# pyannote/pyannote-video

Hardware: AMD Instinct MI355X
Metric: frames/sec end-to-end detect->embed->cluster, 1080p@25fps (higher is better)
Workload: dtype f32 (detector scores, embedder) / f64 (tracker, clustering) / u8 frames; an f16 screening pass with a proven error bound decides which windows the detector's exact f32 chain is evaluated for -- results identical to dense f32 scoring (`dense_scoring`)

## Files before the change

pyannote-video_amd/csrc/ctx.hip:

```cpp
#include "pvf_internal.h"
#include "detect_ml.h"
#include <cmath>
#include <fstream>
#include <mutex>
#include <dlfcn.h>

static thread_local std::string g_err;
void pvf_set_error(const char* msg) { g_err = msg ? msg : ""; }
extern "C" const char* pvf_last_error(void) { return g_err.c_str(); }

static std::mutex g_ctx_mu;
static std::unordered_map<uint64_t, std::unique_ptr<Ctx>> g_ctxs;
static uint64_t g_next_ctx = 0x1000;

Ctx* pvf_ctx(pvf_handle h)
{
    std::lock_guard<std::mutex> lk(g_ctx_mu);
    auto it = g_ctxs.find(h);
    if (it == g_ctxs.end()) throw PvfError("unknown context handle");
    return it->second.get();
}

std::map<std::string, Tensor> pvf_read_container(const char* path)
{
// ... 216 lines not shown
        for (auto& pr : kv.second.pending) {
            float ms = 0;
            if (hipEventElapsedTime(&ms, pr.first, pr.second) == hipSuccess) kv.second.total_ms += ms;
            c->event_pool.push_back(pr.first);
            c->event_pool.push_back(pr.second);
        }
        kv.second.pending.clear();
    }
}

#define API_BEGIN try {
#define API_END                                                        \
    return 0;                                                          \
    }                                                                  \
    catch (const std::exception& e) { pvf_set_error(e.what()); return -1; } \
    catch (...) { pvf_set_error("unknown error"); return -2; }

extern "C" int32_t pvf_version(void) { return 500; }

extern "C" int32_t pvf_device_count(int32_t* n)
{
    API_BEGIN
    int k = 0;
    hipError_t e = hipGetDeviceCount(&k);
    if (e != hipSuccess) k = 0;
    *n = k;
    API_END
}

extern "C" int32_t pvf_ctx_create_prio(int32_t device, int32_t priority_class, pvf_handle* out)
{
    API_BEGIN
    int k = 0;
    if (hipGetDeviceCount(&k) != hipSuccess || k <= 0) throw PvfError("no HIP device visible: libpvface has no CPU fallback");
    PVF_REQUIRE(device >= 0 && device < k, "device index out of range");
    HIP_CHECK(hipSetDevice(device));
    hipDeviceProp_t prop;
    HIP_CHECK(hipGetDeviceProperties(&prop, device));
    if (strncmp(prop.gcnArchName, "gfx950", 6) != 0)
        throw PvfError(std::string("libpvface is built for gfx950 (MI355X) only; device is ") + prop.gcnArchName);
    std::unique_ptr<Ctx> c(new Ctx());
    c->device = device;
    c->n_cu = prop.multiProcessorCount;
    {
        int lo = 0, hi = 0;
        HIP_CHECK(hipDeviceGetStreamPriorityRange(&lo, &hi));
        int prio = priority_class < 0 ? lo : hi;
        if (const char* e = getenv("PVF_MAIN_STREAM_PRIO")) prio = (strcmp(e, "low") == 0) ? lo : hi;
        HIP_CHECK(hipStreamCreateWithPriority(&c->stream, hipStreamNonBlocking, priority_class == 2 ? lo : prio));
        HIP_CHECK(hipStreamCreateWithPriority(&c->det_stream, hipStreamNonBlocking, priority_class == 2 ? hi : lo));
    }
    if (const char* e = getenv("PVF_DETECTOR_SCREENING")) c->det_screen = atoi(e) != 0;
    if (const char* e = getenv("PVF_EMBEDDER_SPLIT")) c->emb_split = atoi(e) != 0;
    std::lock_guard<std::mutex> lk(g_ctx_mu);
    uint64_t id = g_next_ctx++;
    g_ctxs[id] = std::move(c);
    *out = id;
    API_END
}

extern "C" int32_t pvf_ctx_create(int32_t device, pvf_handle* out) { return pvf_ctx_create_prio(device, 0, out); }

extern "C" int32_t pvf_ctx_destroy(pvf_handle h)
{
    API_BEGIN
    Ctx* c = pvf_ctx(h);
    HIP_CHECK(hipSetDevice(c->device));
    (void)hipStreamSynchronize(c->stream);
    (void)hipStreamSynchronize(c->det_stream);
    for (auto& kv : c->frames) if (kv.second.owned) (void)hipFree((void*)kv.second.d);
    for (auto& kv : c->trackers) {
        Tracker& t = *kv.second;
        if (t.share) { if (--*t.share > 0) continue; delete t.share; t.share = nullptr; }
        if (t.d_state) (void)hipFree(t.d_state);
    }
    for (auto p : c->tracker_pool) (void)hipFree(p);
    for (int k = 0; k < 2; ++k) if (c->det_ev[k]) (void)hipEventDestroy(c->det_ev[k]);
    ml_plans_free(c);
    ingest_free_all(c);
    render_free_all(c);
    for (auto& kv : c->frame_pool) for (auto q : kv.second) {
        if (q.free_after) (void)hipEventDestroy(q.free_after);
        if (q.free_after_det) (void)hipEventDestroy(q.free_after_det);
        (void)hipFree(q.p);
    }
    if (c->d_orient_lut) (void)hipFree(c->d_orient_lut);
    if (c->d_wrap_lut) (void)hipFree(c->d_wrap_lut);
    (void)hipStreamDestroy(c->stream);
    (void)hipStreamDestroy(c->det_stream);
    std::lock_guard<std::mutex> lk(g_ctx_mu);
    g_ctxs.erase(h);
    API_END
}

extern "C" int32_t pvf_sync(pvf_handle h)
{
    API_BEGIN
    Ctx* c = pvf_ctx(h);
    std::lock_guard<std::recursive_mutex> det_lock(c->det_mu);
    std::lock_guard<std::recursive_mutex> api_lock(c->api_mu);
    HIP_CHECK(hipStreamSynchronize(c->det_stream));
    HIP_CHECK(hipStreamSynchronize(c->stream));
    API_END
}

extern "C" int32_t pvf_load_detector(pvf_handle h, const char* path)
// ... 219 lines not shown
```

pyannote-video_amd/csrc/pvf_internal.h:

```cpp
#pragma once
#include <hip/hip_runtime.h>
#include <cstdint>
#include <cstdio>
#include <cstring>
#include <deque>
#include <map>
#include <atomic>
#include <memory>
#include <mutex>
#include <stdexcept>
#include <string>
#include <unordered_map>
#include <vector>
#include "../../include/pvface.h"

#define PVF_FHOG_STRIDE 32

struct PvfError : std::runtime_error { using std::runtime_error::runtime_error; };
struct CandOverflow : PvfError { int needed; explicit CandOverflow(int n) : PvfError("detector: candidate buffer overflow"), needed(n) {} };
struct ScreenRetry : PvfError { ScreenRetry() : PvfError("detector: screening pass gave up") {} };

#define HIP_CHECK(expr)                                                                              \
    do {                                                                                             \
        hipError_t _e = (expr);                                                                      \
// ... 160 lines not shown
constexpr size_t TRK_B = TRK_A + (size_t)32 * 64 * 64 * 2;
constexpr size_t TRK_AS = TRK_B + (size_t)64 * 64;
constexpr size_t TRK_BS = TRK_AS + (size_t)512 * 32 * 2;
constexpr size_t TRK_POS = TRK_BS + 32;
constexpr size_t TRK_DOUBLES = TRK_POS + 4;
constexpr size_t TRKF_PLANE = (size_t)64 * 64;
constexpr size_t TRKF_A = 5 * TRKF_PLANE * sizeof(float);
constexpr size_t TRKF_BYTES = TRKF_A + TRKF_PLANE;
#define TRKF_SLOT(q) ((((q) & 511) << 3) | ((q) >> 9))

struct ChipJob {
    const uint8_t* img; int h, w;
    int bx0, by0, sw, sh, levels;
    double m[4], b[2];
    int rows, cols;
    bool empty;
};
struct ChipDetails { double l, t, r, b, cs, sn; int rows, cols; };

struct Ctx {
    int device = 0;
    hipStream_t stream = nullptr;
    hipStream_t det_stream = nullptr;
    DetectorModel det;
    ShapeModel shape;
    EmbedModel emb;
    TrackerTables ttab;
    std::unordered_map<uint64_t, Frame> frames;
    std::unordered_map<uint64_t, std::unique_ptr<Tracker>> trackers;
    std::vector<double*> tracker_pool;
    std::atomic<uint64_t> next_id{1};
    std::recursive_mutex api_mu;
    std::recursive_mutex det_mu;
    std::mutex frames_mu;
    std::mutex prof_mu;
    bool prof_on = false;
    std::map<std::string, ProfFamily> prof;
    std::vector<hipEvent_t> event_pool;
    DevBuf s_grad, s_pyr, s_hist, s_norm, s_feat, s_cand, s_misc, s_chip, s_chip_pyr, s_act0, s_act1, s_act2, s_trk0, s_trk1, s_trk2, s_trkfeat, s_clu0, s_clu1;
    HostBuf h_cand, h_misc;
    StageRing stage;
    DevBuf s_cand2[2], s_fptr[2];
    HostBuf h_cand2[2], h_fptr[2];
    hipEvent_t det_ev[2] = {nullptr, nullptr};
    int det_slot = 0;
    int det_cand_cap = 8192;
    bool det_screen = true, det_screen_suspended = false, screen_attr_set = false;
    int screen_list_cap = 1 << 20;
    DevBuf s_screen;
    int64_t screen_batches = 0, screen_listed = 0, screen_retries = 0;
    double screen_pipe_err = -1;
    bool screen_pipe_flushes_subnormals = false;
    bool emb_split = true, emb_probe_done = false;
    DevBuf s_emb_flags, s_emb_redo;
    int64_t emb_split_faces = 0, emb_reruns = 0;
    double emb_pipe_err = -1;
    int n_cu = 256;
    struct PoolBuf { uint8_t* p; hipEvent_t free_after; hipEvent_t free_after_det; };
    std::map<size_t, std::deque<PoolBuf>> frame_pool;
    size_t frame_pool_bytes = 0;
    void* ingest_rings = nullptr;
    void* render_state = nullptr;
    struct MlPlanCache* ml_plans = nullptr;
    std::map<std::vector<int>, std::unique_ptr<DevBuf>> resize_tabs;
    const void* feat_ring_owner = nullptr;
    uint8_t* d_orient_lut = nullptr;
    uint8_t* d_wrap_lut = nullptr;
    DevBuf s_orb_set, s_orb_work;
    int orb_n = 0, orb_cap = 0;

    Frame frame(uint64_t id)
    {
        std::lock_guard<std::mutex> lk(frames_mu);
        auto it = frames.find(id);
        if (it == frames.end()) throw PvfError("unknown frame handle");
        Frame& f = it->second;
        if (f.ready) {
            HIP_CHECK(hipStreamWaitEvent(stream, f.ready, 0));
            HIP_CHECK(hipStreamWaitEvent(det_stream, f.ready, 0));
            (void)hipEventDestroy(f.ready);
            f.ready = nullptr;
        }
        return f;
    }
    uint8_t* take_frame_buffer(size_t bytes, hipStream_t writer)
    {
        PoolBuf b{nullptr, nullptr, nullptr};
        {
            std::lock_guard<std::mutex> lk(frames_mu);
            auto& v = frame_pool[bytes];
            if (!v.empty()) { b = v.front(); v.pop_front(); frame_pool_bytes -= bytes; }
        }
        if (!b.p) {
            HIP_CHECK(hipMalloc((void**)&b.p, bytes));
            return b.p;
        }
        for (hipEvent_t e : {b.free_after, b.free_after_det}) {
            if (!e) continue;
            if (writer) HIP_CHECK(hipStreamWaitEvent(writer, e, 0));
            else HIP_CHECK(hipEventSynchronize(e));
            (void)hipEventDestroy(e);
        }
        return b.p;
    }
    void pool_give(uint8_t* p, size_t bytes)
    {
        hipEvent_t e = nullptr, e2 = nullptr;
// ... 86 lines not shown
```

pyannote-video_amd/csrc/resnet.hip:

```cpp
#include "pvf_internal.h"
#include <cmath>
#include <cstdlib>
#include <cstring>
#include <vector>

typedef float f32x4 __attribute__((ext_vector_type(4)));
typedef uint32_t u32x4 __attribute__((ext_vector_type(4)));
typedef float f32x16 __attribute__((ext_vector_type(16)));
typedef _Float16 f16x8 __attribute__((ext_vector_type(8)));
typedef _Float16 f16x2 __attribute__((ext_vector_type(2)));
typedef uint32_t u32x2 __attribute__((ext_vector_type(2)));

void face_chip_details(const EmbedModel& m, const int32_t* pts, ChipDetails* out)
{
    const double size = m.chip_size, padding = m.chip_padding;
    double fx[51], fy[51], tx[51], ty[51];
    int n = 0;
    for (int i = 17; i < 68; ++i) {
        if ((55 <= i && i <= 59) || (65 <= i && i <= 67)) continue;
        if (17 <= i && i <= 26) continue;
        fx[n] = ((padding + (double)m.mean_shape[2 * (i - 17)]) / (2 * padding + 1)) * size;
        fy[n] = ((padding + (double)m.mean_shape[2 * (i - 17) + 1]) / (2 * padding + 1)) * size;
        tx[n] = pts[2 * i]; ty[n] = pts[2 * i + 1];
        ++n;
    }
    double mfx = 0, mfy = 0, mtx = 0, mty = 0;
    for (int i = 0; i < n; ++i) { mfx += fx[i]; mfy += fy[i]; mtx += tx[i]; mty += ty[i]; }
    mfx /= n; mfy /= n; mtx /= n; mty /= n;
    double a = 0, b = 0, s = 0;
    for (int i = 0; i < n; ++i) {
        const double ax = fx[i] - mfx, ay = fy[i] - mfy, bx = tx[i] - mtx, by = ty[i] - mty;
        a += ax * bx + ay * by;
        b += ax * by - ay * bx;
        s += ax * ax + ay * ay;
    }
    const double ca = a / s, cb = b / s;
    const double scale = std::sqrt(ca * ca + cb * cb);
    const double hx = size / 2.0, hy = size / 2.0;
    const double cx = (ca * (hx - mfx) - cb * (hy - mfy)) + mtx;
    const double cy = (cb * (hx - mfx) + ca * (hy - mfy)) + mty;
    const double wv = size * scale;
    out->l = cx - wv / 2; out->t = cy - wv / 2; out->r = cx + wv / 2; out->b = cy + wv / 2;
    out->cs = ca / scale; out->sn = cb / scale;
    out->rows = m.chip_size; out->cols = m.chip_size;
}

struct ConvArgs {
    const float* in; int B, H, W, Cin;
    const float* w; int K;
    const float* frag;
    const float* bias; const float* gamma; const float* beta;
    float* out; int OH, OW, Cout;
    int AH, AW;
    int ksz, stride, pad;
    int skip_mode;
    const float* skip; int XH, XW, XC, SH, SW;
    const uint32_t* wsplit; float out_scale; int* flags;
};


__device__ __forceinline__ int small_div(int x, int d, float rd)
{
    int q = (int)((float)x * rd);
    const int r = x - q * d;
    q += (r >= d) ? 1 : 0;
    q -= (r < 0) ? 1 : 0;
    return q;
}

template <int WM, int WN>
__device__ __forceinline__ void conv_epilogue(const ConvArgs& a, float* smem, const f32x16& acc0, const f32x16& acc1, long M, long m0, int n0,
                                              int rel0, int b_first, int hw, float r_hw, float r_ow, int wave, int lane)
{
    constexpr int PITCH = 36;
    const int wm = wave / WN, wn = wave % WN;
    const int li = lane & 31, kh = lane >> 5;
    const int col = n0 + wn * 32 + li;
    const float bias = a.bias[col], g = a.gamma[col], bt = a.beta[col];
    if (a.AH == a.OH && a.AW == a.OW && a.skip_mode != 2) {
        float* T = smem + wave * 64 * PITCH;
#pragma unroll
        for (int t = 0; t < 2; ++t)
#pragma unroll
            for (int reg = 0; reg < 16; ++reg)
                T[(t * 32 + (reg & 3) + 8 * (reg >> 2) + 4 * kh) * PITCH + li] = (t == 0 ? acc0[reg] : acc1[reg]);
        __builtin_amdgcn_wave_barrier();
        const int c4 = lane & 7, cb = n0 + wn * 32 + 4 * c4;
        const float4 bias4 = *reinterpret_cast<const float4*>(a.bias + cb), g4 = *reinterpret_cast<const float4*>(a.gamma + cb),
                     bt4 = *reinterpret_cast<const float4*>(a.beta + cb);
#pragma unroll
        for (int it = 0; it < 8; ++it) {
            const int row = it * 8 + (lane >> 3);
            const long m = m0 + wm * 64 + row;
            if (m >= M) continue;
            const float4 x = *reinterpret_cast<const float4*>(&T[row * PITCH + 4 * c4]);
            float4 v = make_float4((x.x + bias4.x) * g4.x + bt4.x, (x.y + bias4.y) * g4.y + bt4.y, (x.z + bias4.z) * g4.z + bt4.z,
                                   (x.w + bias4.w) * g4.w + bt4.w);
            if (a.skip_mode == 1) {
                const float4 sk = *reinterpret_cast<const float4*>(a.skip + (size_t)m * a.Cout + cb);
                v.x += sk.x; v.y += sk.y; v.z += sk.z; v.w += sk.w;
            }
            { v.x = v.x < 0.0f ? 0.0f : v.x; v.y = v.y < 0.0f ? 0.0f : v.y; v.z = v.z < 0.0f ? 0.0f : v.z; v.w = v.w < 0.0f ? 0.0f : v.w; }
            *reinterpret_cast<float4*>(a.out + (size_t)m * a.Cout + cb) = v;
        }
        return;
    }
#pragma unroll
    for (int t = 0; t < 2; ++t)
#pragma unroll
        for (int reg = 0; reg < 16; ++reg) {
            const int row = (reg & 3) + 8 * (reg >> 2) + 4 * kh;
            const long m = m0 + wm * 64 + t * 32 + row;
            if (m >= M) continue;
            const int rel = rel0 + wm * 64 + t * 32 + row;
            const int bb = small_div(rel, hw, r_hw);
            const int rem = rel - bb * hw;
            const int oy = small_div(rem, a.OW, r_ow);
            const int ox = rem - oy * a.OW;
            const int b = b_first + bb;
            float v = 0.0f;
            if (oy < a.AH && ox < a.AW) v = ((t == 0 ? acc0[reg] : acc1[reg]) + bias) * g + bt;
            if (a.skip_mode == 1) v += a.skip[(size_t)m * a.Cout + col];
            else if (a.skip_mode == 2) {
                if (col < a.XC && oy < a.SH && ox < a.SW) {
                    const float* q = a.skip + (((size_t)b * a.XH + 2 * oy) * a.XW + 2 * ox) * a.XC + col;
                    v += (((q[0] + q[a.XC]) + q[(size_t)a.XW * a.XC]) + q[(size_t)a.XW * a.XC + a.XC]) * 0.25f;
                }
            }
            if (v < 0.0f) v = 0.0f;
            a.out[(size_t)m * a.Cout + col] = v;
        }
}

template <int WM, int WN>
__global__ void __launch_bounds__(256) conv_mfma_k(ConvArgs a)
{
    constexpr int BM = 64 * WM, BN = 32 * WN, KC = 32, PITCH = 36;
    static_assert(WM * WN == 4, "four waves per block");
    constexpr int SM_ROWS = (BM + BN > 256) ? BM + BN : 256;
    __shared__ __attribute__((aligned(16))) float smem[SM_ROWS * PITCH];
    float* As = smem;
    float* Bs = smem + BM * PITCH;
    const int tid = threadIdx.x, lane = tid & 63, wave = tid >> 6;
    const int wm = wave / WN, wn = wave % WN;
    const long M = (long)a.B * a.OH * a.OW;
    const long m0 = (long)blockIdx.x * BM;
    const int n0 = blockIdx.y * BN;
    f32x16 acc0, acc1;
#pragma unroll
    for (int i = 0; i < 16; ++i) { acc0[i] = 0.0f; acc1[i] = 0.0f; }

    constexpr int A_F4 = BM * 8 / 256, B_F4 = BN * 8 / 256;
    constexpr int RSRC_FLAGS = 0x00020000;
    constexpr int OOB = (int)0x80000000;
    const int hw = a.OH * a.OW;
    const int b_first = (int)(m0 / hw);
    const int rel0 = (int)(m0 - (long)b_first * hw);
    const float r_hw = 1.0f / (float)hw, r_ow = 1.0f / (float)a.OW;
    const size_t face = (size_t)a.H * a.W * a.Cin;
    const size_t in_bytes = (size_t)(a.B - b_first) * face * sizeof(float);
    const __amdgpu_buffer_rsrc_t rs_in = __builtin_amdgcn_make_buffer_rsrc((void*)(a.in + (size_t)b_first * face), 0,
                                                                           in_bytes > 0x7ffffff0u ? 0x7ffffff0 : (int)in_bytes, RSRC_FLAGS);
    int pa_off[A_F4], pa_y[A_F4], pa_x[A_F4];
#pragma unroll
    for (int q = 0; q < A_F4; ++q) {
        const int i = (tid + q * 256) >> 3;
        const long m = m0 + i;
        pa_off[q] = 0; pa_y[q] = -(1 << 20); pa_x[q] = 0;
        if (m < M) {
            const int rel = rel0 + i;
            const int bb = small_div(rel, hw, r_hw);
            const int rem = rel - bb * hw;
            const int oy = small_div(rem, a.OW, r_ow);
            const int ox = rem - oy * a.OW;
            if (oy < a.AH && ox < a.AW) {
                pa_y[q] = oy * a.stride - a.pad; pa_x[q] = ox * a.stride - a.pad;
                pa_off[q] = ((bb * a.H + pa_y[q]) * a.W + pa_x[q]) * a.Cin;
            }
        }
    }
    const int Kpad = (a.K + KC - 1) / KC * KC;
    const int j4 = tid & 7;
    const float* wrow[B_F4];
// ... 18 lines not shown
        if (f_k + KC < Kpad) {
            f_k += KC;
            f_c += KC;
            if (f_c >= a.Cin) { f_c = 0; if (++f_s == a.ksz) { f_s = 0; ++f_r; } }
        }
    };
    auto issue = [&]() {
#pragma unroll
        for (int q = 0; q < A_F4; ++q) va[q] = __builtin_amdgcn_raw_buffer_load_b128(rs_in, voff[q], 0, 0);
#pragma unroll
        for (int q = 0; q < B_F4; ++q) vb[q] = *reinterpret_cast<const float4*>(wrow[q] + woff);
    };
    auto park = [&]() {
#pragma unroll
        for (int q = 0; q < A_F4; ++q) {
            uint32_t* row = reinterpret_cast<uint32_t*>(&As[((tid + q * 256) >> 3) * PITCH + 2 * j4]);
            *reinterpret_cast<uint2*>(row) = make_uint2(va[q].x, va[q].z);
            *reinterpret_cast<uint2*>(row + 16) = make_uint2(va[q].y, va[q].w);
        }
#pragma unroll
        for (int q = 0; q < B_F4; ++q) {
            float* row = &Bs[((tid + q * 256) >> 3) * PITCH + 2 * j4];
            *reinterpret_cast<float2*>(row) = make_float2(vb[q].x, vb[q].z);
            *reinterpret_cast<float2*>(row + 16) = make_float2(vb[q].y, vb[q].w);
        }
    };
    const int li = lane & 31, kh = lane >> 5;
    const float* pa0 = &As[(wm * 64 + li) * PITCH + 16 * kh];
    const float* pa1 = pa0 + 32 * PITCH;
    const float* pb = &Bs[(wn * 32 + li) * PITCH + 16 * kh];
    offsets();
    issue();
    offsets();
    for (int k0 = 0; k0 < Kpad; k0 += KC) {
        park();
        __syncthreads();
        issue();
        __builtin_amdgcn_sched_barrier(0);
        offsets();
        f32x4 fa0[4], fa1[4], fb[4];
#pragma unroll
        for (int q = 0; q < 4; ++q) {
            fa0[q] = *reinterpret_cast<const f32x4*>(pa0 + 4 * q);
            fa1[q] = *reinterpret_cast<const f32x4*>(pa1 + 4 * q);
            fb[q] = *reinterpret_cast<const f32x4*>(pb + 4 * q);
        }
#pragma unroll
        for (int s = 0; s < 16; ++s) {
            acc0 = __builtin_amdgcn_mfma_f32_32x32x2f32(fa0[s >> 2][s & 3], fb[s >> 2][s & 3], acc0, 0, 0, 0);
            acc1 = __builtin_amdgcn_mfma_f32_32x32x2f32(fa1[s >> 2][s & 3], fb[s >> 2][s & 3], acc1, 0, 0, 0);
        }
        __syncthreads();
    }
    conv_epilogue<WM, WN>(a, smem, acc0, acc1, M, m0, n0, rel0, b_first, hw, r_hw, r_ow, wave, lane);
}


#define EMB_A_SCALE_EXP 8
#define EMB_F16_LIMIT 65504.0f

__global__ void __launch_bounds__(256) conv_wsplit_k(const float* __restrict__ w, int total, int w_exp, _Float16* __restrict__ out)
{
    const int i = blockIdx.x * 256 + threadIdx.x;
    if (i >= total) return;
    const float v = ldexpf(w[i], w_exp);
    const _Float16 hi = (_Float16)v;
    const _Float16 lo = (_Float16)(v - (float)hi);
    const int row32 = i >> 5, kk = i & 31;
    out[(size_t)row32 * 64 + kk] = hi;
    out[(size_t)row32 * 64 + 32 + kk] = lo;
}

template <int WM, int WN>
__global__ void __launch_bounds__(256) conv_split_k(ConvArgs a)
{
    constexpr int BM = 64 * WM, BN = 32 * WN, KC = 32, PITCH = 36;
    static_assert(WM * WN == 4, "four waves per block");
    constexpr int SM_ROWS = (BM + BN > 256) ? BM + BN : 256;
    __shared__ __attribute__((aligned(16))) float smem[SM_ROWS * PITCH];
    uint32_t* As = reinterpret_cast<uint32_t*>(smem);
    uint32_t* Bs = As + BM * PITCH;
    const int tid = threadIdx.x, lane = tid & 63, wave = tid >> 6;
    const int wm = wave / WN, wn = wave % WN;
    const long M = (long)a.B * a.OH * a.OW;
    const long m0 = (long)blockIdx.x * BM;
    const int n0 = blockIdx.y * BN;
    f32x16 acc0, acc1;
#pragma unroll
    for (int i = 0; i < 16; ++i) { acc0[i] = 0.0f; acc1[i] = 0.0f; }

    constexpr int A_F4 = BM * 8 / 256, B_F4 = BN * 8 / 256;
    constexpr int RSRC_FLAGS = 0x00020000;
    constexpr int OOB = (int)0x80000000;
    const int hw = a.OH * a.OW;
    const int b_first = (int)(m0 / hw);
    const int rel0 = (int)(m0 - (long)b_first * hw);
    const float r_hw = 1.0f / (float)hw, r_ow = 1.0f / (float)a.OW;
    const size_t face = (size_t)a.H * a.W * a.Cin;
    const size_t in_bytes = (size_t)(a.B - b_first) * face * sizeof(float);
    const __amdgpu_buffer_rsrc_t rs_in = __builtin_amdgcn_make_buffer_rsrc((void*)(a.in + (size_t)b_first * face), 0,
                                                                           in_bytes > 0x7ffffff0u ? 0x7ffffff0 : (int)in_bytes, RSRC_FLAGS);
    int pa_off[A_F4], pa_y[A_F4], pa_x[A_F4];
#pragma unroll
    for (int q = 0; q < A_F4; ++q) {
        const int i = (tid + q * 256) >> 3;
        const long m = m0 + i;
        pa_off[q] = 0; pa_y[q] = -(1 << 20); pa_x[q] = 0;
        if (m < M) {
            const int rel = rel0 + i;
            const int bb = small_div(rel, hw, r_hw);
            const int rem = rel - bb * hw;
            const int oy = small_div(rem, a.OW, r_ow);
            const int ox = rem - oy * a.OW;
            if (oy < a.AH && ox < a.AW) {
                pa_y[q] = oy * a.stride - a.pad; pa_x[q] = ox * a.stride - a.pad;
                pa_off[q] = ((bb * a.H + pa_y[q]) * a.W + pa_x[q]) * a.Cin;
            }
        }
    }
    const int Kpad = (a.K + KC - 1) / KC * KC;
    const int j4 = tid & 7;
    const u32x4* wrow[B_F4];
#pragma unroll
    for (int q = 0; q < B_F4; ++q) wrow[q] = reinterpret_cast<const u32x4*>(a.wsplit) + (size_t)(n0 + ((tid + q * 256) >> 3)) * (Kpad / 4) + j4;
    u32x4 va[A_F4], vb[B_F4];
    int f_r = 0, f_s = 0, f_c = 0, f_k = 0;
    int voff[A_F4], woff = 0;
    auto offsets = [&]() {
        const int kq = f_k + 4 * j4;
        const int r = f_r, sft = f_s;
        const int delta = (r * a.W + sft) * a.Cin + f_c + 4 * j4;
        const int k_ok = (kq < a.K) ? -1 : 0;
#pragma unroll
        for (int q = 0; q < A_F4; ++q) {
            const int iy = pa_y[q] + r, ix = pa_x[q] + sft;
            const int ok = k_ok & -(int)((unsigned)iy < (unsigned)a.H) & -(int)((unsigned)ix < (unsigned)a.W);
            voff[q] = (((pa_off[q] + delta) * 4) & ok) | (OOB & ~ok);
        }
        woff = f_k / 4;
        if (f_k + KC < Kpad) {
            f_k += KC;
            f_c += KC;
            if (f_c >= a.Cin) { f_c = 0; if (++f_s == a.ksz) { f_s = 0; ++f_r; } }
        }
    };
    auto issue = [&]() {
#pragma unroll
        for (int q = 0; q < A_F4; ++q) va[q] = __builtin_amdgcn_raw_buffer_load_b128(rs_in, voff[q], 0, 0);
#pragma unroll
        for (int q = 0; q < B_F4; ++q) vb[q] = wrow[q][woff];
    };
    const float sa = (float)(1 << EMB_A_SCALE_EXP);
    auto park = [&]() {
        int bad = 0;
#pragma unroll
        for (int q = 0; q < A_F4; ++q) {
            const f32x4 xv = __builtin_bit_cast(f32x4, va[q]) * sa;
            const float x0 = xv.x, x1 = xv.y, x2 = xv.z, x3 = xv.w;
            const int ok = (int)(fabsf(x0) < EMB_F16_LIMIT) & (int)(fabsf(x1) < EMB_F16_LIMIT) & (int)(fabsf(x2) < EMB_F16_LIMIT) &
                           (int)(fabsf(x3) < EMB_F16_LIMIT);
            bad |= ok ? 0 : (1 << q);
            const _Float16 h0 = (_Float16)x0, h1 = (_Float16)x1, h2 = (_Float16)x2, h3 = (_Float16)x3;
            const f16x2 h01 = {h0, h1}, h23 = {h2, h3};
            const f16x2 l01 = {(_Float16)(x0 - (float)h0), (_Float16)(x1 - (float)h1)};
            const f16x2 l23 = {(_Float16)(x2 - (float)h2), (_Float16)(x3 - (float)h3)};
            uint32_t* row = &As[((tid + q * 256) >> 3) * PITCH + 2 * j4];
            *reinterpret_cast<u32x2*>(row) = (u32x2){__builtin_bit_cast(uint32_t, h01), __builtin_bit_cast(uint32_t, h23)};
            *reinterpret_cast<u32x2*>(row + 16) = (u32x2){__builtin_bit_cast(uint32_t, l01), __builtin_bit_cast(uint32_t, l23)};
        }
#pragma unroll
        for (int q = 0; q < B_F4; ++q) *reinterpret_cast<u32x4*>(&Bs[((tid + q * 256) >> 3) * PITCH + 4 * j4]) = vb[q];
        if (bad)
            for (int q = 0; q < A_F4; ++q)
                if ((bad >> q) & 1) a.flags[b_first + small_div(rel0 + ((tid + q * 256) >> 3), hw, r_hw)] = 1;
    };
    const int li = lane & 31, kh = lane >> 5;
    const uint32_t* pa0 = &As[(wm * 64 + li) * PITCH + 4 * kh];
    const uint32_t* pa1 = pa0 + 32 * PITCH;
    const uint32_t* pb = &Bs[(wn * 32 + li) * PITCH + 4 * kh];
    offsets();
    issue();
    offsets();
    for (int k0 = 0; k0 < Kpad; k0 += KC) {
        park();
        __syncthreads();
        issue();
        __builtin_amdgcn_sched_barrier(0);
        offsets();
#pragma unroll
        for (int s = 0; s < 2; ++s) {
            const f16x8 ah0 = *reinterpret_cast<const f16x8*>(pa0 + 8 * s), al0 = *reinterpret_cast<const f16x8*>(pa0 + 16 + 8 * s);
            const f16x8 ah1 = *reinterpret_cast<const f16x8*>(pa1 + 8 * s), al1 = *reinterpret_cast<const f16x8*>(pa1 + 16 + 8 * s);
            const f16x8 bh = *reinterpret_cast<const f16x8*>(pb + 8 * s), bl = *reinterpret_cast<const f16x8*>(pb + 16 + 8 * s);
            acc0 = __builtin_amdgcn_mfma_f32_32x32x16_f16(ah0, bh, acc0, 0, 0, 0);
            acc1 = __builtin_amdgcn_mfma_f32_32x32x16_f16(ah1, bh, acc1, 0, 0, 0);
            acc0 = __builtin_amdgcn_mfma_f32_32x32x16_f16(ah0, bl, acc0, 0, 0, 0);
            acc1 = __builtin_amdgcn_mfma_f32_32x32x16_f16(ah1, bl, acc1, 0, 0, 0);
            acc0 = __builtin_amdgcn_mfma_f32_32x32x16_f16(al0, bh, acc0, 0, 0, 0);
            acc1 = __builtin_amdgcn_mfma_f32_32x32x16_f16(al1, bh, acc1, 0, 0, 0);
        }
        __syncthreads();
    }
#pragma unroll
    for (int i = 0; i < 16; ++i) { acc0[i] *= a.out_scale; acc1[i] *= a.out_scale; }
    conv_epilogue<WM, WN>(a, smem, acc0, acc1, M, m0, n0, rel0, b_first, hw, r_hw, r_ow, wave, lane);
}

__global__ void __launch_bounds__(64) embed_probe_k(const uint4* __restrict__ a, const uint4* __restrict__ b, int steps, float* __restrict__ d)
{
    const int lane = threadIdx.x;
    f32x16 acc;
#pragma unroll
    for (int i = 0; i < 16; ++i) acc[i] = 0.0f;
    for (int s = 0; s < steps; ++s)
        acc = __builtin_amdgcn_mfma_f32_32x32x16_f16(__builtin_bit_cast(f16x8, a[s * 64 + lane]), __builtin_bit_cast(f16x8, b[s * 64 + lane]), acc, 0, 0, 0);
    for (int i = 0; i < 16; ++i) d[lane * 16 + i] = acc[i];
}

#define STEM_ROWS 4
#define STEM_IN_DW 1464
#define STEM_NP 77
__global__ void __launch_bounds__(64) stem_frag_k(const float* __restrict__ w, float* __restrict__ frag)
{
    const int p = blockIdx.x, l = threadIdx.x;
    const int r = p / 11, t = 2 * (p - r * 11) + (l >> 5);
    frag[p * 64 + l] = (t < 21) ? w[(size_t)(l & 31) * 224 + (r * 7 + t / 3) * 4 + t % 3] : 0.0f;
}

__global__ void __launch_bounds__(192) stem_conv_k(const uint8_t* __restrict__ chips, int B, const float* __restrict__ frag, const float* __restrict__ bias,
                                                   const float* __restrict__ gamma, const float* __restrict__ beta, float* __restrict__ out)
{
    constexpr int S = 150, OW = 72;
    __shared__ uint32_t s_in[STEM_IN_DW];
    __shared__ __attribute__((aligned(16))) float s_b[STEM_NP * 64];
    const int tid = threadIdx.x, lane = tid & 63, wave = tid >> 6;
    const int face = blockIdx.y, oy0 = blockIdx.x * STEM_ROWS;
    {
        const size_t total = (size_t)B * S * S * 3;
        const __amdgpu_buffer_rsrc_t rs = __builtin_amdgcn_make_buffer_rsrc((void*)(chips + (size_t)face * S * S * 3), 0,
                                                                             (int)std::min<size_t>(total - (size_t)face * S * S * 3, 0x7ffffff0u), 0x00020000);
        const int first = 2 * oy0 * S * 3;
        for (int i = tid; i < STEM_IN_DW; i += 192) s_in[i] = __builtin_amdgcn_raw_buffer_load_b32(rs, 4 * i, first, 0);
        const float4* f4 = reinterpret_cast<const float4*>(frag);
        float4* b4 = reinterpret_cast<float4*>(s_b);
        for (int i = tid; i < STEM_NP * 16; i += 192) b4[i] = f4[i];
    }
    __syncthreads();
    const int li = lane & 31, kh = lane >> 5;
    const uint8_t* px = reinterpret_cast<const uint8_t*>(s_in);
    const uint8_t* base[3];
#pragma unroll
    for (int t = 0; t < 3; ++t) {
        const int m = (wave * 3 + t) * 32 + li;
        const int oy = m / OW, ox = m - oy * OW;
        base[t] = px + ((2 * oy) * S + 2 * ox) * 3 + kh;
    }
    const float M0 = 122.782f, M1 = 117.001f, M2 = 104.298f;
    const float mean3[3] = {kh ? M1 : M0, kh ? M0 : M2, kh ? M2 : M1};
// ... 145 lines not shown
                    const float y = (acc[t][reg] + bs) * g + bt;
                    x[t][reg] = y < 0.0f ? 0.0f : y;
                }
        }
#pragma unroll
        for (int t = 0; t < 2; ++t)
#pragma unroll
            for (int reg = 0; reg < 16; ++reg)
                __builtin_amdgcn_raw_buffer_store_b32(__builtin_bit_cast(uint32_t, x[t][reg]), ro, e_off[t][reg], 0, 0);
        __syncthreads();
        item = next;
    }
}

__global__ void __launch_bounds__(256) maxpool3s2_k(const float* __restrict__ in, int B, int H, int W, int C, float* __restrict__ out, int OH, int OW)
{
    const size_t i = (size_t)blockIdx.x * blockDim.x + threadIdx.x;
    const size_t total = (size_t)B * OH * OW * C;
    if (i >= total) return;
    const int c = (int)(i % C);
    size_t t = i / C;
    const int ox = (int)(t % OW); t /= OW;
    const int oy = (int)(t % OH);
    const int b = (int)(t / OH);
    float mx = -INFINITY;
    for (int r = 0; r < 3; ++r)
        for (int s = 0; s < 3; ++s) {
            const float v = in[(((size_t)b * H + oy * 2 + r) * W + ox * 2 + s) * C + c];
            mx = fmaxf(mx, v);
        }
    out[i] = mx;
}

__global__ void __launch_bounds__(256) head_k(const float* __restrict__ x, int HW, const float* __restrict__ fc, float* __restrict__ out)
{
    __shared__ float feat[256];
    const int b = blockIdx.x, t = threadIdx.x;
    float s = 0.0f;
    for (int i = 0; i < HW; ++i) s += x[((size_t)b * HW + i) * 256 + t];
    feat[t] = s / (float)HW;
    __syncthreads();
    if (t < 128) {
        float acc = 0.0f;
        for (int o = 0; o < 256; ++o) acc += feat[o] * fc[(size_t)o * 128 + t];
        out[(size_t)b * 128 + t] = acc;
    }
}

static void launch_conv(Ctx* c, const ConvArgs& a)
{
    const long M = (long)a.B * a.OH * a.OW;
    PVF_REQUIRE(a.Cin % 32 == 0, "conv: input channels must be a multiple of 32 (the 3-channel first layer has a kernel of its own: stem_conv_k)");
    PVF_REQUIRE(a.OH * a.OW < (1 << 21) && a.Cout % 32 == 0, "conv: output map too large for the kernel's index arithmetic / Cout not a multiple of 32");
    if (a.frag && a.Cin == 32 && a.Cout == 32 && a.H == 35 && a.W == 35 && a.OH == 35 && a.OW == 35 && a.AH == 35 && a.AW == 35 && a.ksz == 3 &&
        a.stride == 1 && a.pad == 1 && a.skip_mode != 2) {
        static std::atomic<uint64_t> attr_set{0};
        const size_t lds = (size_t)(C32_TILE_FLOATS + 144 * 64) * sizeof(float);
        const uint64_t bit = 1ull << (c->device & 63);
        if (!(attr_set.load() & bit)) {
            HIP_CHECK(hipFuncSetAttribute(reinterpret_cast<const void*>(conv3x3_c32_k), hipFuncAttributeMaxDynamicSharedMemorySize, (int)lds));
            attr_set.fetch_or(bit);
        }
        const int items = a.B * (35 / C32_ROWS);
        hipLaunchKernelGGL(conv3x3_c32_k, dim3((unsigned)std::min(items, 2 * c->n_cu)), dim3(256), lds, c->stream, a.in, a.frag, a.bias, a.gamma, a.beta,
                           a.skip_mode == 1 ? a.skip : nullptr, a.out, items);
    } else if (a.Cout == 32) {
        const dim3 grid((unsigned)((M + 255) / 256), 1);
        if (a.wsplit) hipLaunchKernelGGL((conv_split_k<4, 1>), grid, dim3(256), 0, c->stream, a);
        else hipLaunchKernelGGL((conv_mfma_k<4, 1>), grid, dim3(256), 0, c->stream, a);
    } else {
        PVF_REQUIRE(a.Cout % 64 == 0, "conv: Cout must be 32 or a multiple of 64");
        const dim3 grid((unsigned)((M + 127) / 128), a.Cout / 64);
        if (a.wsplit) hipLaunchKernelGGL((conv_split_k<2, 2>), grid, dim3(256), 0, c->stream, a);
        else hipLaunchKernelGGL((conv_mfma_k<2, 2>), grid, dim3(256), 0, c->stream, a);
    }
}

void conv_layer_upload(ConvLayer& L, const float* w, const float* bias, const float* gamma, const float* beta)
{
    const int cin = L.cin, cout = L.cout, k = L.k;
    const int cp = (cin == 3) ? 4 : cin;
    const int K = k * k * cp, Kpad = (K + 31) / 32 * 32;
    std::vector<float> wt((size_t)cout * Kpad, 0.0f);
    for (int o = 0; o < cout; ++o)
        for (int ci = 0; ci < cin; ++ci)
            for (int r = 0; r < k; ++r)
                for (int s = 0; s < k; ++s) {
                    const int kk = (r * k + s) * cp + ci;
                    wt[(size_t)o * Kpad + kk] = w[(((size_t)o * cin + ci) * k + r) * k + s];
                }
    auto up = [](const float* src, size_t count) {
        float* d = nullptr;
        HIP_CHECK(hipMalloc((void**)&d, count * sizeof(float)));
        HIP_CHECK(hipMemcpy(d, src, count * sizeof(float), hipMemcpyHostToDevice));
        return d;
    };
    L.d_w = up(wt.data(), wt.size());
    float wmax = 0.0f;
    for (float v : wt) wmax = std::max(wmax, std::fabs(v));
    int ex = 0;
    if (wmax > 0.0f && std::isfinite(wmax)) { std::frexp(wmax, &ex); L.w_exp = 15 - ex; }
    L.d_bias = up(bias, cout);
    L.d_gamma = up(gamma, cout);
    L.d_beta = up(beta, cout);
}

void conv_layer_free(ConvLayer& L)
{
    for (void* p : {(void*)L.d_w, (void*)L.d_bias, (void*)L.d_gamma, (void*)L.d_beta, (void*)L.d_frag, (void*)L.d_wsplit})
        if (p) (void)hipFree(p);
    L.d_w = L.d_bias = L.d_gamma = L.d_beta = L.d_frag = nullptr;
    L.d_wsplit = nullptr;
}

static void conv_bind_weights(Ctx* c, ConvLayer& L, bool split, bool generic, int* flags, ConvArgs& a)
{
    a.w = L.d_w; a.K = L.k * L.k * L.cin; a.bias = L.d_bias; a.gamma = L.d_gamma; a.beta = L.d_beta;
    a.frag = nullptr; a.wsplit = nullptr; a.out_scale = 0.0f; a.flags = nullptr;
    const bool own = !generic && L.cin == 32 && L.cout == 32 && L.k == 3;
    if (own) {
        if (!L.d_frag) {
            HIP_CHECK(hipMalloc(&L.d_frag, 144 * 64 * sizeof(float)));
            hipLaunchKernelGGL(conv_frag_k, dim3(144), dim3(64), 0, c->stream, L.d_w, 288, L.d_frag);
        }
        a.frag = L.d_frag;
        return;
// ... 41 lines not shown
                           steps, d_d);
        HIP_CHECK(hipMemcpyAsync(hd, d_d, sizeof hd, hipMemcpyDeviceToHost, c->stream));
        HIP_CHECK(hipStreamSynchronize(c->stream));
        double worst = 0;
        for (int l = 0; l < 64; ++l)
            for (int i = 0; i < 16; ++i) {
                const int col = l & 31, row = (i & 3) + 8 * (i >> 2) + 4 * (l >> 5);
                double ex = 0, mag = 0;
                for (int k = 0; k < K; ++k) { const double t = A[(size_t)row * K + k] * B[(size_t)k * 32 + col]; ex += t; mag += std::fabs(t); }
                worst = std::max(worst, std::fabs((double)hd[l * 16 + i] - ex) / (mag > 0 ? mag : 1.0));
            }
        return worst;
    };
    auto put = [&](int r, int k, int col, float av, float bv) {
        ha[ia(r, k)] = f16_bits(av); hb[ia(col, k)] = f16_bits(bv);
        A[(size_t)r * K + k] = (double)(_Float16)av; B[(size_t)k * 32 + col] = (double)(_Float16)bv;
    };
    double worst = 0;
    for (int k = 0; k < K; ++k)
        for (int r = 0; r < 32; ++r) {
            const float av = (float)((rnd() < 0.5 ? -1 : 1) * std::ldexp(1.0 + rnd(), (int)(rnd() * 25) - 10));
            const float bv = (float)((rnd() < 0.5 ? -1 : 1) * std::ldexp(1.0 + rnd(), (int)(rnd() * 25) - 10));
            put(r, k, r, av, bv);
        }
    worst = std::max(worst, run());
    for (int k = 0; k < K; ++k)
        for (int r = 0; r < 32; ++r) {
            const float x = (float)(rnd() * 2048.0), w = (float)((rnd() * 2 - 1) * 32768.0);
            const _Float16 xh = (_Float16)x, wh = (_Float16)w;
            const float xl = x - (float)xh, wl = w - (float)wh;
            const int term = (k >> 4) % 3;
            put(r, k, r, term == 2 ? xl : (float)xh, term == 1 ? wl : (float)wh);
        }
    worst = std::max(worst, run());
    (void)hipFree(dev);
    c->emb_pipe_err = worst;
    PVF_REQUIRE(worst <= (double)K * std::ldexp(1.0, -22),
                "embed_probe: v_mfma_f32_32x32x16_f16 does not place or accumulate as the split embedder (conv_split_k) assumes on this device");
}

static void resnet_run(Ctx* c, const uint8_t* d_chips, int n, float* h_out, bool split, int* h_flags, const EmbedTap* tap = nullptr)
{
    const EmbedModel& e = c->emb;
    PVF_REQUIRE(e.loaded, "embedder not loaded");
    const int S = e.chip_size;
    const int MAXB = 4096;
    const int h1 = 1 + (S - 7) / 2;
    const int hp = 1 + (h1 - 3) / 2;
    const int cap = std::min(n, MAXB);
    const size_t big = (size_t)cap * h1 * h1 * 32;
    c->s_act0.ensure(std::max(big, (size_t)cap * S * S * 4) * sizeof(float));
    c->s_act1.ensure(big * sizeof(float));
    c->s_act2.ensure((size_t)cap * hp * hp * 32 * sizeof(float) + (size_t)cap * 128 * sizeof(float));
    PVF_REQUIRE(!tap || n <= MAXB, "embedder stage access: at most 4096 faces");
    auto tapped = [&](int stage, const float* d, int B, int H, int W, int C) {
        if (tap && tap->stage == stage && tap->h_out)
            HIP_CHECK(hipMemcpyAsync(tap->h_out, d, (size_t)B * H * W * C * sizeof(float), hipMemcpyDeviceToHost, c->stream));
    };
    for (int b0 = 0; b0 < n; b0 += MAXB) {
        const int B = std::min(MAXB, n - b0);
        ProfScope ps(c, "conv");
        float* x = c->s_act0.as<float>();
        float* y = c->s_act1.as<float>();
        float* z = c->s_act2.as<float>();
        const ConvLayer& L0 = e.convs[0];
        PVF_REQUIRE(S == 150 && L0.cout == 32 && L0.k == 7 && h1 == 72, "stem kernel: 150 x 150 chips, 7 x 7 stride 2, 32 channels");
        if (!c->emb.d_stem) {
            HIP_CHECK(hipMalloc(&c->emb.d_stem, STEM_NP * 64 * sizeof(float)));
            hipLaunchKernelGGL(stem_frag_k, dim3(STEM_NP), dim3(64), 0, c->stream, L0.d_w, c->emb.d_stem);
        }
        hipLaunchKernelGGL(stem_conv_k, dim3(h1 / STEM_ROWS, B), dim3(192), 0, c->stream, d_chips + (size_t)b0 * S * S * 3, B, c->emb.d_stem,
                           L0.d_bias, L0.d_gamma, L0.d_beta, y);
        tapped(0, y, B, h1, h1, 32);
        ConvArgs a;
        const size_t npool = (size_t)B * hp * hp * 32;
        hipLaunchKernelGGL(maxpool3s2_k, dim3((unsigned)((npool + 255) / 256)), dim3(256), 0, c->stream, y, B, h1, h1, 32, z, hp, hp);
        tapped(1, z, B, hp, hp, 32);
        float* cur = z; float* t1 = x; float* t2 = y;
        int H = hp, W = hp;
        static const int UN[14][3] = {{32, 32, 0}, {32, 32, 0}, {32, 32, 0}, {32, 64, 1}, {64, 64, 0}, {64, 64, 0}, {64, 64, 0},
                                      {64, 128, 1}, {128, 128, 0}, {128, 128, 0}, {128, 256, 1}, {256, 256, 0}, {256, 256, 0}, {256, 256, 1}};
        int* flags = nullptr;
        if (split) {
            flags = c->s_emb_flags.as<int>();
            HIP_CHECK(hipMemsetAsync(flags, 0, (size_t)B * sizeof(int), c->stream));
        }
        for (int u = 0; u < 14; ++u) {
            const int cin = UN[u][0], nn = UN[u][1], down = UN[u][2];
            ConvLayer& La = c->emb.convs[1 + 2 * u];
            ConvLayer& Lb = c->emb.convs[2 + 2 * u];
            const int stride = down ? 2 : 1, pad = down ? 0 : 1;
            const int ah = 1 + (H + 2 * pad - 3) / stride, aw = 1 + (W + 2 * pad - 3) / stride;
            memset(&a, 0, sizeof a);
            a.in = cur; a.B = B; a.H = H; a.W = W; a.Cin = cin;
            a.out = t1; a.OH = ah; a.OW = aw; a.Cout = nn; a.AH = ah; a.AW = aw; a.ksz = 3; a.stride = stride; a.pad = pad; a.skip_mode = 0;
            conv_bind_weights(c, La, split, false, flags, a);
            launch_conv(c, a);
            tapped(2 + 2 * u, t1, B, ah, aw, nn);
            int sh = H, sw = W;
            if (down) { sh = 1 + (H - 2) / 2; sw = 1 + (W - 2) / 2; }
            const int oh = std::max(ah, sh), ow = std::max(aw, sw);
            memset(&a, 0, sizeof a);
            a.in = t1; a.B = B; a.H = ah; a.W = aw; a.Cin = nn;
            a.out = t2; a.OH = oh; a.OW = ow; a.Cout = nn; a.AH = ah; a.AW = aw; a.ksz = 3; a.stride = 1; a.pad = 1;
            a.skip_mode = down ? 2 : 1; a.skip = cur; a.XH = H; a.XW = W; a.XC = cin; a.SH = sh; a.SW = sw;
            conv_bind_weights(c, Lb, split, false, flags, a);
            launch_conv(c, a);
            tapped(3 + 2 * u, t2, B, oh, ow, nn);
            float* old = cur; cur = t2; t2 = old;
            H = oh; W = ow;
        }
        float* d_out = reinterpret_cast<float*>(c->s_act2.as<uint8_t>() + (size_t)cap * hp * hp * 32 * sizeof(float));
        hipLaunchKernelGGL(head_k, dim3(B), dim3(256), 0, c->stream, cur, H * W, e.d_fc, d_out);
        HIP_CHECK(hipGetLastError());
        HIP_CHECK(hipMemcpyAsync(h_out + (size_t)b0 * 128, d_out, (size_t)B * 128 * sizeof(float), hipMemcpyDeviceToHost, c->stream));
        if (split) HIP_CHECK(hipMemcpyAsync(h_flags + b0, flags, (size_t)B * sizeof(int), hipMemcpyDeviceToHost, c->stream));
    }
    HIP_CHECK(hipStreamSynchronize(c->stream));
}

void resnet_forward(Ctx* c, const uint8_t* d_chips, int n, float* h_out)
{
    if (!c->emb_split) { resnet_run(c, d_chips, n, h_out, false, nullptr); return; }
    if (!c->emb_probe_done) { embed_probe(c); c->emb_probe_done = true; }
    c->s_emb_flags.ensure((size_t)std::min(n, 4096) * sizeof(int));
    std::vector<int> flags(n, 0);
    resnet_run(c, d_chips, n, h_out, true, flags.data());
    c->emb_split_faces += n;
    std::vector<int> redo;
    for (int i = 0; i < n; ++i) if (flags[i]) redo.push_back(i);
    if (redo.empty()) return;
    c->emb_reruns += (int64_t)redo.size();
    const size_t chip = (size_t)150 * 150 * 3;
    c->s_emb_redo.ensure(redo.size() * chip);
    uint8_t* d = c->s_emb_redo.as<uint8_t>();
    for (size_t j = 0; j < redo.size(); ++j)
        HIP_CHECK(hipMemcpyAsync(d + j * chip, d_chips + (size_t)redo[j] * chip, chip, hipMemcpyDeviceToDevice, c->stream));
    std::vector<float> e(redo.size() * 128);
    resnet_run(c, d, (int)redo.size(), e.data(), false, nullptr);
    for (size_t j = 0; j < redo.size(); ++j) memcpy(h_out + (size_t)redo[j] * 128, e.data() + j * 128, 128 * sizeof(float));
}

void resnet_debug_stage(Ctx* c, const uint8_t* d_chips, int n, bool split, EmbedTap* tap, int* h_flags)
{
    PVF_REQUIRE(tap && tap->stage >= 0 && tap->stage < EMB_STAGES, "pvf_debug_embed_stage: stage must be 0..29");
    {
        int H = 72, C = 32;
        if (tap->stage >= 1) H = 35;
        for (int u = 0; 2 + 2 * u <= tap->stage; ++u) {
            static const int UN[14][2] = {{32, 0}, {32, 0}, {32, 0}, {64, 1}, {64, 0}, {64, 0}, {64, 0}, {128, 1}, {128, 0}, {128, 0}, {256, 1}, {256, 0}, {256, 0}, {256, 1}};
            C = UN[u][0];
            const int a = UN[u][1] ? 1 + (H - 3) / 2 : H, s = UN[u][1] ? 1 + (H - 2) / 2 : H;
            H = (tap->stage == 2 + 2 * u) ? a : std::max(a, s);
        }
        tap->dims[0] = H; tap->dims[1] = H; tap->dims[2] = C;
    }
    if (!tap->h_out) return;
    if (split) c->s_emb_flags.ensure((size_t)std::min(n, 4096) * sizeof(int));
    std::vector<float> desc((size_t)n * 128);
    std::vector<int> flags(n, 0);
    resnet_run(c, d_chips, n, desc.data(), split, flags.data(), tap);
// ... 79 lines not shown
```

Measured before the change: 4635.

## Emit pre-split f16 hi/lo packed activations from conv epilogue for split embedder path

The split-precision conv kernels now have a templated epilogue that can also write activations already converted to scaled f16 hi/lo pairs in the kernel's packed layout. Range overflow is flagged per face in the epilogue. Downstream conv_split_k instances then load these packed tiles straight into shared memory, skipping the per-tile f32-to-f16 split and range checks. This removes repeated conversion work and also drops the f32 write of the first conv in each unit, except when a tap needs it. The cost is an extra packed-activation buffer, more epilogue stores, and more complex buffer aliasing between the f32 and packed forms.

```diff
diff --git a/pyannote-video_amd/csrc/ctx.hip b/pyannote-video_amd/csrc/ctx.hip
--- a/pyannote-video_amd/csrc/ctx.hip
+++ b/pyannote-video_amd/csrc/ctx.hip
@@ -292,6 +292,7 @@
     }
     if (const char* e = getenv("PVF_DETECTOR_SCREENING")) c->det_screen = atoi(e) != 0;
     if (const char* e = getenv("PVF_EMBEDDER_SPLIT")) c->emb_split = atoi(e) != 0;
+    if (const char* e = getenv("PVF_EMBEDDER_PACKED")) c->emb_packed = atoi(e) != 0;
     std::lock_guard<std::mutex> lk(g_ctx_mu);
     uint64_t id = g_next_ctx++;
     g_ctxs[id] = std::move(c);
diff --git a/pyannote-video_amd/csrc/pvf_internal.h b/pyannote-video_amd/csrc/pvf_internal.h
--- a/pyannote-video_amd/csrc/pvf_internal.h
+++ b/pyannote-video_amd/csrc/pvf_internal.h
@@ -236,7 +236,9 @@
     double screen_pipe_err = -1;
     bool screen_pipe_flushes_subnormals = false;
     bool emb_split = true, emb_probe_done = false;
+    bool emb_packed = true;
     DevBuf s_emb_flags, s_emb_redo;
+    DevBuf s_act_pk;
     int64_t emb_split_faces = 0, emb_reruns = 0;
     double emb_pipe_err = -1;
     int n_cu = 256;
diff --git a/pyannote-video_amd/csrc/resnet.hip b/pyannote-video_amd/csrc/resnet.hip
--- a/pyannote-video_amd/csrc/resnet.hip
+++ b/pyannote-video_amd/csrc/resnet.hip
@@ -56,7 +56,11 @@
     int skip_mode;
     const float* skip; int XH, XW, XC, SH, SW;
     const uint32_t* wsplit; float out_scale; int* flags;
+    int in_pk; uint32_t* out_pk;
 };
+
+#define EMB_A_SCALE_EXP 8
+#define EMB_F16_LIMIT 65504.0f
 
 
 __device__ __forceinline__ int small_div(int x, int d, float rd)
@@ -68,7 +72,7 @@
     return q;
 }
 
-template <int WM, int WN>
+template <int WM, int WN, bool PKOUT>
 __device__ __forceinline__ void conv_epilogue(const ConvArgs& a, float* smem, const f32x16& acc0, const f32x16& acc1, long M, long m0, int n0,
                                               int rel0, int b_first, int hw, float r_hw, float r_ow, int wave, int lane)
 {
@@ -101,7 +105,21 @@
                 v.x += sk.x; v.y += sk.y; v.z += sk.z; v.w += sk.w;
             }
             { v.x = v.x < 0.0f ? 0.0f : v.x; v.y = v.y < 0.0f ? 0.0f : v.y; v.z = v.z < 0.0f ? 0.0f : v.z; v.w = v.w < 0.0f ? 0.0f : v.w; }
-            *reinterpret_cast<float4*>(a.out + (size_t)m * a.Cout + cb) = v;
+            if (!PKOUT || a.out) *reinterpret_cast<float4*>(a.out + (size_t)m * a.Cout + cb) = v;
+            if (PKOUT && a.out_pk) {
+                const float sa = (float)(1 << EMB_A_SCALE_EXP);
+                const float x0 = v.x * sa, x1 = v.y * sa, x2 = v.z * sa, x3 = v.w * sa;
+                const int ok = (int)(fabsf(x0) < EMB_F16_LIMIT) & (int)(fabsf(x1) < EMB_F16_LIMIT) & (int)(fabsf(x2) < EMB_F16_LIMIT) &
+                               (int)(fabsf(x3) < EMB_F16_LIMIT);
+                const _Float16 h0 = (_Float16)x0, h1 = (_Float16)x1, h2 = (_Float16)x2, h3 = (_Float16)x3;
+                const f16x2 h01 = {h0, h1}, h23 = {h2, h3};
+                const f16x2 l01 = {(_Float16)(x0 - (float)h0), (_Float16)(x1 - (float)h1)};
+                const f16x2 l23 = {(_Float16)(x2 - (float)h2), (_Float16)(x3 - (float)h3)};
+                uint32_t* p = a.out_pk + ((size_t)m * (a.Cout >> 5) + (cb >> 5)) * 32 + ((cb & 31) >> 1);
+                *reinterpret_cast<u32x2*>(p) = (u32x2){__builtin_bit_cast(uint32_t, h01), __builtin_bit_cast(uint32_t, h23)};
+                *reinterpret_cast<u32x2*>(p + 16) = (u32x2){__builtin_bit_cast(uint32_t, l01), __builtin_bit_cast(uint32_t, l23)};
+                if (!ok) a.flags[b_first + small_div(rel0 + wm * 64 + row, hw, r_hw)] = 1;
+            }
         }
         return;
     }
@@ -128,7 +146,15 @@
                 }
             }
             if (v < 0.0f) v = 0.0f;
-            a.out[(size_t)m * a.Cout + col] = v;
+            if (!PKOUT || a.out) a.out[(size_t)m * a.Cout + col] = v;
+            if (PKOUT && a.out_pk) {
+                const float x = v * (float)(1 << EMB_A_SCALE_EXP);
+                if (!(fabsf(x) < EMB_F16_LIMIT)) a.flags[b] = 1;
+                const _Float16 h = (_Float16)x, l = (_Float16)(x - (float)h);
+                _Float16* p = reinterpret_cast<_Float16*>(a.out_pk) + ((size_t)m * (a.Cout >> 5) + (col >> 5)) * 64 + (col & 31);
+                p[0] = h;
+                p[32] = l;
+            }
         }
 }
 
@@ -253,12 +279,9 @@
         }
         __syncthreads();
     }
-    conv_epilogue<WM, WN>(a, smem, acc0, acc1, M, m0, n0, rel0, b_first, hw, r_hw, r_ow, wave, lane);
-}
-
-
-#define EMB_A_SCALE_EXP 8
-#define EMB_F16_LIMIT 65504.0f
+    conv_epilogue<WM, WN, false>(a, smem, acc0, acc1, M, m0, n0, rel0, b_first, hw, r_hw, r_ow, wave, lane);
+}
+
 
 __global__ void __launch_bounds__(256) conv_wsplit_k(const float* __restrict__ w, int total, int w_exp, _Float16* __restrict__ out)
 {
@@ -272,7 +295,7 @@
     out[(size_t)row32 * 64 + 32 + kk] = lo;
 }
 
-template <int WM, int WN>
+template <int WM, int WN, bool PK>
 __global__ void __launch_bounds__(256) conv_split_k(ConvArgs a)
 {
     constexpr int BM = 64 * WM, BN = 32 * WN, KC = 32, PITCH = 36;
@@ -353,6 +376,13 @@
     };
     const float sa = (float)(1 << EMB_A_SCALE_EXP);
     auto park = [&]() {
+        if constexpr (PK) {
+#pragma unroll
+            for (int q = 0; q < A_F4; ++q) *reinterpret_cast<u32x4*>(&As[((tid + q * 256) >> 3) * PITCH + 4 * j4]) = va[q];
+#pragma unroll
+            for (int q = 0; q < B_F4; ++q) *reinterpret_cast<u32x4*>(&Bs[((tid + q * 256) >> 3) * PITCH + 4 * j4]) = vb[q];
+            return;
+        }
         int bad = 0;
 #pragma unroll
         for (int q = 0; q < A_F4; ++q) {
@@ -404,7 +434,7 @@
     }
 #pragma unroll
     for (int i = 0; i < 16; ++i) { acc0[i] *= a.out_scale; acc1[i] *= a.out_scale; }
-    conv_epilogue<WM, WN>(a, smem, acc0, acc1, M, m0, n0, rel0, b_first, hw, r_hw, r_ow, wave, lane);
+    conv_epilogue<WM, WN, true>(a, smem, acc0, acc1, M, m0, n0, rel0, b_first, hw, r_hw, r_ow, wave, lane);
 }
 
 __global__ void __launch_bounds__(64) embed_probe_k(const uint4* __restrict__ a, const uint4* __restrict__ b, int steps, float* __restrict__ d)
@@ -656,6 +686,8 @@
     const long M = (long)a.B * a.OH * a.OW;
     PVF_REQUIRE(a.Cin % 32 == 0, "conv: input channels must be a multiple of 32 (the 3-channel first layer has a kernel of its own: stem_conv_k)");
     PVF_REQUIRE(a.OH * a.OW < (1 << 21) && a.Cout % 32 == 0, "conv: output map too large for the kernel's index arithmetic / Cout not a multiple of 32");
+    PVF_REQUIRE(!(a.in_pk || a.out_pk) || (a.wsplit && a.flags && !a.frag && a.Cout % 64 == 0), "conv: packed activations are the split kernel's (Cout a multiple of 64)");
+    PVF_REQUIRE(a.out || a.out_pk, "conv: no output tensor");
     if (a.frag && a.Cin == 32 && a.Cout == 32 && a.H == 35 && a.W == 35 && a.OH == 35 && a.OW == 35 && a.AH == 35 && a.AW == 35 && a.ksz == 3 &&
         a.stride == 1 && a.pad == 1 && a.skip_mode != 2) {
         static std::atomic<uint64_t> attr_set{0};
@@ -670,12 +702,13 @@
                            a.skip_mode == 1 ? a.skip : nullptr, a.out, items);
     } else if (a.Cout == 32) {
         const dim3 grid((unsigned)((M + 255) / 256), 1);
-        if (a.wsplit) hipLaunchKernelGGL((conv_split_k<4, 1>), grid, dim3(256), 0, c->stream, a);
+        if (a.wsplit) hipLaunchKernelGGL((conv_split_k<4, 1, false>), grid, dim3(256), 0, c->stream, a);
         else hipLaunchKernelGGL((conv_mfma_k<4, 1>), grid, dim3(256), 0, c->stream, a);
     } else {
         PVF_REQUIRE(a.Cout % 64 == 0, "conv: Cout must be 32 or a multiple of 64");
         const dim3 grid((unsigned)((M + 127) / 128), a.Cout / 64);
-        if (a.wsplit) hipLaunchKernelGGL((conv_split_k<2, 2>), grid, dim3(256), 0, c->stream, a);
+        if (a.wsplit && a.in_pk) hipLaunchKernelGGL((conv_split_k<2, 2, true>), grid, dim3(256), 0, c->stream, a);
+        else if (a.wsplit) hipLaunchKernelGGL((conv_split_k<2, 2, false>), grid, dim3(256), 0, c->stream, a);
         else hipLaunchKernelGGL((conv_mfma_k<2, 2>), grid, dim3(256), 0, c->stream, a);
     }
 }
@@ -823,6 +856,9 @@
     c->s_act0.ensure(std::max(big, (size_t)cap * S * S * 4) * sizeof(float));
     c->s_act1.ensure(big * sizeof(float));
     c->s_act2.ensure((size_t)cap * hp * hp * 32 * sizeof(float) + (size_t)cap * 128 * sizeof(float));
+    const bool packed = split && c->emb_packed;
+    const size_t pk_bytes = (size_t)cap * 17 * 17 * 64 * sizeof(float);
+    if (packed) c->s_act_pk.ensure(pk_bytes);
     PVF_REQUIRE(!tap || n <= MAXB, "embedder stage access: at most 4096 faces");
     auto tapped = [&](int stage, const float* d, int B, int H, int W, int C) {
         if (tap && tap->stage == stage && tap->h_out)
@@ -848,6 +884,7 @@
         hipLaunchKernelGGL(maxpool3s2_k, dim3((unsigned)((npool + 255) / 256)), dim3(256), 0, c->stream, y, B, h1, h1, 32, z, hp, hp);
         tapped(1, z, B, hp, hp, 32);
         float* cur = z; float* t1 = x; float* t2 = y;
+        uint32_t* cur_pk = nullptr;
         int H = hp, W = hp;
         static const int UN[14][3] = {{32, 32, 0}, {32, 32, 0}, {32, 32, 0}, {32, 64, 1}, {64, 64, 0}, {64, 64, 0}, {64, 64, 0},
                                       {64, 128, 1}, {128, 128, 0}, {128, 128, 0}, {128, 256, 1}, {256, 256, 0}, {256, 256, 0}, {256, 256, 1}};
@@ -863,21 +900,30 @@
             const int stride = down ? 2 : 1, pad = down ? 0 : 1;
             const int ah = 1 + (H + 2 * pad - 3) / stride, aw = 1 + (W + 2 * pad - 3) / stride;
             memset(&a, 0, sizeof a);
-            a.in = cur; a.B = B; a.H = H; a.W = W; a.Cin = cin;
+            const bool unit_pk = packed && !(cin == 32 && nn == 32);
+            const bool tap_a = tap && tap->stage == 2 + 2 * u && tap->h_out;
+            a.in = cur_pk ? reinterpret_cast<const float*>(cur_pk) : cur; a.in_pk = cur_pk != nullptr;
+            a.B = B; a.H = H; a.W = W; a.Cin = cin;
             a.out = t1; a.OH = ah; a.OW = aw; a.Cout = nn; a.AH = ah; a.AW = aw; a.ksz = 3; a.stride = stride; a.pad = pad; a.skip_mode = 0;
+            if (unit_pk) { a.out_pk = reinterpret_cast<uint32_t*>(t1); a.out = tap_a ? t2 : nullptr; }
             conv_bind_weights(c, La, split, false, flags, a);
             launch_conv(c, a);
-            tapped(2 + 2 * u, t1, B, ah, aw, nn);
+            tapped(2 + 2 * u, unit_pk ? t2 : t1, B, ah, aw, nn);
             int sh = H, sw = W;
             if (down) { sh = 1 + (H - 2) / 2; sw = 1 + (W - 2) / 2; }
             const int oh = std::max(ah, sh), ow = std::max(aw, sw);
             memset(&a, 0, sizeof a);
-            a.in = t1; a.B = B; a.H = ah; a.W = aw; a.Cin = nn;
+            a.in = t1; a.in_pk = unit_pk; a.B = B; a.H = ah; a.W = aw; a.Cin = nn;
             a.out = t2; a.OH = oh; a.OW = ow; a.Cout = nn; a.AH = ah; a.AW = aw; a.ksz = 3; a.stride = 1; a.pad = 1;
             a.skip_mode = down ? 2 : 1; a.skip = cur; a.XH = H; a.XW = W; a.XC = cin; a.SH = sh; a.SW = sw;
+            if (unit_pk && u + 1 < 14) {
+                PVF_REQUIRE((size_t)B * oh * ow * nn * sizeof(float) <= pk_bytes, "embedder: packed arena too small");
+                a.out_pk = c->s_act_pk.as<uint32_t>();
+            }
             conv_bind_weights(c, Lb, split, false, flags, a);
             launch_conv(c, a);
             tapped(3 + 2 * u, t2, B, oh, ow, nn);
+            cur_pk = a.out_pk;
             float* old = cur; cur = t2; t2 = old;
             H = oh; W = ow;
         }
```

Result: no change. 4722 (median of 5 runs) (+1.9%).
